# ray-project/ray

Hardware: AMD Instinct MI355X
Metric: train_samples_per_sec (higher is better)
Workload: dtype bf16; 1 GPU; model=llama3-8b, global_batch=8, micro_batch=8, seq_len=4096, parallelism=dp1, n_params=8030261248, bucket_mb=128, grad_checkpoint=False, harness=ray_amd.train.TorchTrainer

## Files before the change

ray_amd/csrc/hip/gemm_wgrad.hip:

```cpp
#include "common.h"
#include "fa_bwd_lds_layout.h"

typedef __attribute__((ext_vector_type(8))) __bf16 wg_bf16x8;
typedef __attribute__((ext_vector_type(16))) float wg_f32x16;
typedef __attribute__((ext_vector_type(2))) unsigned int wg_u32x2;
typedef __attribute__((ext_vector_type(4))) unsigned int wg_u32x4;

#define WG_STAGE 65536
#define WG_HALF 16384
#define WG_B 32768

template <int OFF>
DEV_INLINE wg_u32x2 wg_tr(unsigned addr) {
  wg_u32x2 v;
  asm volatile("ds_read_b64_tr_b16 %0, %1 offset:%2"
               : "=v"(v)
               : "v"(addr), "n"(OFF)
               : "memory");
  return v;
}

DEV_INLINE wg_bf16x8 wg_frag(wg_u32x2 lo, wg_u32x2 hi) {
  wg_u32x4 t = __builtin_shufflevector(lo, hi, 0, 1, 2, 3);
  return __builtin_bit_cast(wg_bf16x8, t);
}

DEV_INLINE void wg_stage_half(const char* g, unsigned lane_off, char* lds) {
  typedef const __attribute__((address_space(1))) void* gptr;
  typedef __attribute__((address_space(3))) void* lptr;
  __builtin_amdgcn_global_load_lds((gptr)(g + lane_off), (lptr)lds, 16, 0, 0);
  __builtin_amdgcn_global_load_lds((gptr)(g + 128 + lane_off),
                                   (lptr)(lds + 1024), 16, 0, 0);
}

struct WgRegs {
  wg_f32x16 acc[2][2][2];
  wg_u32x2 a[2][4][2];
  wg_u32x2 b[4][2];
};

template <int BASE, int S>
DEV_INLINE void wg_read_a1(WgRegs& r, unsigned a0, unsigned a1) {
  r.a[0][S][0] = wg_tr<BASE + 4096 * S>(a0);
  r.a[0][S][1] = wg_tr<BASE + 4096 * S + 2048>(a1);
  r.a[1][S][0] = wg_tr<BASE + 4096 * S + 512>(a0);
  r.a[1][S][1] = wg_tr<BASE + 4096 * S + 2048 + 512>(a1);
}
template <int BASE>
DEV_INLINE void wg_read_a(WgRegs& r, unsigned a0, unsigned a1) {
  wg_read_a1<BASE, 0>(r, a0, a1);
  wg_read_a1<BASE, 1>(r, a0, a1);
  wg_read_a1<BASE, 2>(r, a0, a1);
  wg_read_a1<BASE, 3>(r, a0, a1);
}

template <int BASE, int S>
DEV_INLINE void wg_read_b1(WgRegs& r, unsigned b0, unsigned b1) {
  r.b[S][0] = wg_tr<BASE + 4096 * S>(b0);
  r.b[S][1] = wg_tr<BASE + 4096 * S + 2048>(b1);
}
template <int BASE>
DEV_INLINE void wg_read_b(WgRegs& r, unsigned b0, unsigned b1) {
  wg_read_b1<BASE, 0>(r, b0, b1);
  wg_read_b1<BASE, 1>(r, b0, b1);
  wg_read_b1<BASE, 2>(r, b0, b1);
  wg_read_b1<BASE, 3>(r, b0, b1);
}

template <int HA, int HB>
DEV_INLINE void wg_mma(WgRegs& r) {
  asm volatile("s_waitcnt lgkmcnt(0)" ::: "memory");
  __builtin_amdgcn_sched_barrier(0);
  __builtin_amdgcn_s_barrier();
  __builtin_amdgcn_sched_barrier(0);
  __builtin_amdgcn_s_setprio(1);
#pragma unroll
  for (int s = 0; s < 4; ++s) {
    const wg_bf16x8 bf = wg_frag(r.b[s][0], r.b[s][1]);
#pragma unroll
    for (int i = 0; i < 2; ++i)
      r.acc[HA][HB][i] = __builtin_amdgcn_mfma_f32_32x32x16_bf16(
          wg_frag(r.a[i][s][0], r.a[i][s][1]), bf, r.acc[HA][HB][i], 0, 0, 0);
  }
  __builtin_amdgcn_s_setprio(0);
  __builtin_amdgcn_sched_barrier(0);
  __builtin_amdgcn_s_barrier();
  __builtin_amdgcn_sched_barrier(0);
}

template <int ST, bool NEXT_B0, bool NEXT2, int VMC>
DEV_INLINE void wg_tile(WgRegs& r, const unsigned (&ra)[2][2],
                        const unsigned (&rb)[2][2], char* lds_w, const char* gA,
                        const char* gB, unsigned la, unsigned lb,
                        long long tileA, long long tileB, int t) {
  constexpr int S = ST * WG_STAGE;
  constexpr int O = (ST ^ 1) * WG_STAGE;
  wg_read_a<0>(r, ra[ST][0], ra[ST][1]);
  wg_read_b<0>(r, rb[ST][0], rb[ST][1]);
  if (NEXT_B0)
    wg_stage_half(gB + (t + 1) * tileB, lb, lds_w + O + WG_B);
  wg_mma<0, 0>(r);
  wg_read_b<WG_HALF>(r, rb[ST][0], rb[ST][1]);
  if (NEXT2) wg_stage_half(gA + (t + 2) * tileA, la, lds_w + S);
  wg_mma<0, 1>(r);
  wg_read_a<WG_HALF>(r, ra[ST][0], ra[ST][1]);
  if (NEXT2)
    wg_stage_half(gB + (t + 2) * tileB + 256, lb, lds_w + S + WG_B + WG_HALF);
  wg_mma<1, 1>(r);
  wg_read_b<0>(r, rb[ST][0], rb[ST][1]);
  if (NEXT2)
    wg_stage_half(gA + (t + 2) * tileA + 256, la, lds_w + S + WG_HALF);
  if (VMC == 6) asm volatile("s_waitcnt vmcnt(6)" ::: "memory");
  if (VMC == 0) asm volatile("s_waitcnt vmcnt(0)" ::: "memory");
  wg_mma<1, 0>(r);
}

template <bool STAGGER>
__global__ __launch_bounds__(512) void gemm_wgrad_bf16(
    const short* __restrict__ dy0, const short* __restrict__ dy1,
    const short* __restrict__ x, short* __restrict__ out0,
    short* __restrict__ out1, int M, long long ldy, long long ldx,
    long long ldo, int NT, int nt0, int KT) {
  __shared__ __attribute__((aligned(1024))) char smem[2 * WG_STAGE];

  const int tid = threadIdx.x;
  const int w = __builtin_amdgcn_readfirstlane(tid >> 6);
  const int lane = tid & 63;
  const int wr = w >> 2, wc = w & 3;

  int tn, tk;
  {
    const int nwg = NT * KT;
    const int orig = blockIdx.x;
    const int xcd = orig & 7;
    const int q = nwg >> 3, rr = nwg & 7;
    const int id = (xcd < rr ? xcd * (q + 1) : rr * (q + 1) + (xcd - rr) * q) +
                   (orig >> 3);
    const int per = 8 * KT;
    const int grp = id / per;
    const int first = grp * 8;
    const int gsz = min(NT - first, 8);
    const int in = id - grp * per;
    tn = first + in % gsz;
    tk = in / gsz;
  }
  const bool p1 = tn >= nt0;
  const short* dy = p1 ? dy1 : dy0;
  short* out = p1 ? out1 : out0;
  const int tn_l = p1 ? tn - nt0 : tn;

  const char* gA = reinterpret_cast<const char*>(dy + (long long)tn_l * 256);
  const char* gB = reinterpret_cast<const char*>(x + (long long)tk * 256);
  const long long tileA = 64 * ldy * 2, tileB = 64 * ldx * 2;

  unsigned la, lb;
  {
    const int r7 = (lane >> 2) & 7;
    const int xo = 2 * (w & 1) + (r7 >> 2);
    const int ch = 4 * (lane >> 5) + ((lane & 3) ^ xo);
    const int row = 8 * w + r7;
    la = (unsigned)(row * (int)ldy * 2 + 16 * ch);
    lb = (unsigned)(row * (int)ldx * 2 + 16 * ch);
  }
  char* const lds_w = smem + 2048 * w;

  const unsigned sm0 = (unsigned)(size_t)(
      (__attribute__((address_space(3))) char*)smem);
  unsigned ra[2][2], rb[2][2];
#pragma unroll
  for (int mm = 0; mm < 2; ++mm) {
    const unsigned tb = sm0 + 2 * fb6_tbase(lane, mm);
    ra[0][mm] = tb + 1024 * wr;
    ra[1][mm] = tb + 1024 * wr + WG_STAGE;
    rb[0][mm] = tb + 512 * wc + WG_B;
    rb[1][mm] = tb + 512 * wc + WG_B + WG_STAGE;
  }

  WgRegs r;
#pragma unroll
  for (int a = 0; a < 2; ++a)
#pragma unroll
    for (int b = 0; b < 2; ++b)
#pragma unroll
      for (int i = 0; i < 2; ++i) r.acc[a][b][i] = wg_f32x16{};

  const int nt = M >> 6;

  wg_stage_half(gA, la, lds_w);
  wg_stage_half(gB, lb, lds_w + WG_B);
  wg_stage_half(gB + 256, lb, lds_w + WG_B + WG_HALF);
  wg_stage_half(gA + 256, la, lds_w + WG_HALF);
  wg_stage_half(gA + tileA, la, lds_w + WG_STAGE);
  wg_stage_half(gB + tileB + 256, lb, lds_w + WG_STAGE + WG_B + WG_HALF);
  wg_stage_half(gA + tileA + 256, la, lds_w + WG_STAGE + WG_HALF);
  asm volatile("s_waitcnt vmcnt(6)" ::: "memory");
  __builtin_amdgcn_s_barrier();
  __builtin_amdgcn_sched_barrier(0);
  if (STAGGER && wr) __builtin_amdgcn_s_barrier();
  __builtin_amdgcn_sched_barrier(0);

  int t = 0;
  for (; t < nt - 2; t += 2) {
    wg_tile<0, true, true, 6>(r, ra, rb, lds_w, gA, gB, la, lb, tileA, tileB,
                              t);
    wg_tile<1, true, true, 6>(r, ra, rb, lds_w, gA, gB, la, lb, tileA, tileB,
                              t + 1);
  }
  wg_tile<0, true, false, 0>(r, ra, rb, lds_w, gA, gB, la, lb, tileA, tileB,
                             t);
  wg_tile<1, false, false, -1>(r, ra, rb, lds_w, gA, gB, la, lb, tileA, tileB,
                               t + 1);
  if (STAGGER && !wr) __builtin_amdgcn_s_barrier();
  __builtin_amdgcn_sched_barrier(0);

  short* const ep = reinterpret_cast<short*>(smem);
  const int hi = lane >> 5, c32 = lane & 31;
#pragma unroll
  for (int ha = 0; ha < 2; ++ha) {
#pragma unroll
    for (int hb = 0; hb < 2; ++hb)
#pragma unroll
      for (int i = 0; i < 2; ++i)
#pragma unroll
        for (int g = 0; g < 16; ++g) {
          const int row = 64 * wr + 32 * i + (g & 3) + 8 * (g >> 2) + 4 * hi;
          const int col = 128 * hb + 32 * wc + c32;
          ep[row * 256 + col] =
              __builtin_bit_cast(short, (__bf16)r.acc[ha][hb][i][g]);
        }
    __syncthreads();
#pragma unroll
    for (int it = 0; it < 8; ++it) {
      const int c = tid + 512 * it;
      const int row = c >> 5, ch = c & 31;
      const short8 v = *reinterpret_cast<const short8*>(ep + row * 256 + 8 * ch);
      *reinterpret_cast<short8*>(
          out + ((long long)tn_l * 256 + 128 * ha + row) * ldo +
          (long long)tk * 256 + 8 * ch) = v;
    }
    __syncthreads();
  }
}
```

ray_amd/csrc/ops.hip:

```cpp
#include <torch/extension.h>
#include <ATen/hip/HIPContext.h>

#include "hip/rmsnorm.hip"
#include "hip/elementwise.hip"
#include "hip/rl_scans.hip"
#include "hip/cross_entropy.hip"
#include "hip/flash_attn_v5.hip"
#include "hip/flash_attn_v7.hip"
#include "hip/fa_bwd_prep.hip"
#include "hip/fa_bwd_v3.hip"
#include "hip/fa_bwd_dq_v5.hip"
#include "hip/fa_bwd_dkv_v6.hip"
#include "hip/gemv.hip"
#include "hip/paged_attn.hip"
#include "hip/paged_attn_prefill.hip"
#include "hip/gemm_wgrad.hip"

#define CHECK_IN(x)                                                     \
  TORCH_CHECK(x.is_cuda(), #x " must be on GPU");                       \
  TORCH_CHECK(x.is_contiguous(), #x " must be contiguous")

static inline hipStream_t cur_stream() {
  return at::hip::getCurrentHIPStream().stream();
}
// ... 273 lines not shown
              "paged cache must be [num_pages, Hkv, 16, D] matching q/k");
  return fp8;
}

static bool check_paged_attn(const at::Tensor& k_cache,
                             const at::Tensor& v_cache,
                             const at::Tensor& block_table, int B, int Hq,
                             int D, double k_scale, double v_scale, int* Hkv) {
  TORCH_CHECK(D == 64 || D == 128, "paged_attn: head_dim must be 64 or 128");
  TORCH_CHECK(k_cache.dim() == 4, "k_cache must be [num_pages, Hkv, 16, D]");
  *Hkv = (int)k_cache.size(1);
  const bool fp8 = check_paged_cache(k_cache, v_cache, *Hkv, D, k_scale,
                                     v_scale);
  TORCH_CHECK(*Hkv >= 1 && Hq % *Hkv == 0, "GQA requires Hq % Hkv == 0");
  const int rep = Hq / *Hkv;
  TORCH_CHECK(rep == 1 || rep == 2 || rep == 4 || rep == 8,
              "paged_attn: Hq/Hkv must be 1, 2, 4 or 8");
  TORCH_CHECK(block_table.dim() == 2 && block_table.size(0) == B &&
              block_table.size(1) >= 1,
              "block_table must be [B, max_pages]");
  return fp8;
}

static void launch_paged_reduce(const at::Tensor& ws, at::Tensor& out, int B,
                                int Hq, int D, int S) {
  const float* ws_o = ws.data_ptr<float>();
  const float* ws_ml = ws_o + (long long)B * Hq * S * D;
  hipLaunchKernelGGL(paged_attn_reduce_bf16, dim3(Hq, B), dim3(D), 0,
                     cur_stream(), ws_o, ws_ml, (short*)out.data_ptr(), Hq, S,
                     D);
}

at::Tensor paged_attn_reduce(at::Tensor workspace, int64_t B, int64_t Hq,
                             int64_t D, int64_t num_splits) {
  CHECK_IN(workspace);
  TORCH_CHECK(workspace.scalar_type() == at::kFloat, "workspace must be fp32");
  TORCH_CHECK(D == 64 || D == 128, "paged_attn: head_dim must be 64 or 128");
  TORCH_CHECK(B >= 1 && B <= 65535 && Hq >= 1 && Hq <= 65535 &&
              num_splits >= 1, "paged_attn_reduce: bad B/Hq/num_splits");
  TORCH_CHECK(workspace.numel() >= B * Hq * num_splits * (D + 2),
              "paged_attn: workspace too small");
  auto out = at::empty({B, Hq, D}, workspace.options().dtype(at::kBFloat16));
  launch_paged_reduce(workspace, out, (int)B, (int)Hq, (int)D,
                      (int)num_splits);
  return out;
}

template <int D, int REP, bool FP8, int EPL>
static void launch_paged_decode(const at::Tensor& q, const at::Tensor& kc,
                                const at::Tensor& vc, const at::Tensor& bt,
                                const at::Tensor& sl, at::Tensor& out,
                                float* ws_o, float* ws_ml, int S, int Hkv,
                                float k_scale, float v_scale) {
  int B = (int)q.size(0);
  hipLaunchKernelGGL((paged_attn_decode_kernel<D, REP, FP8, EPL>),
                     dim3(S, Hkv, B), dim3(256), 0, cur_stream(),
                     (const short*)q.data_ptr(), (const void*)kc.data_ptr(),
                     (const void*)vc.data_ptr(), bt.data_ptr<int>(),
                     sl.data_ptr<int>(), (short*)out.data_ptr(), ws_o, ws_ml,
                     Hkv, (int)kc.size(0), (int)bt.size(1),
                     1.4426950408889634f / sqrtf((float)D) * k_scale,
                     v_scale);
}

at::Tensor paged_attn_decode(at::Tensor q, at::Tensor k_cache,
                             at::Tensor v_cache, at::Tensor block_table,
                             at::Tensor seq_lens, int64_t num_splits,
                             c10::optional<at::Tensor> workspace,
                             double k_scale, double v_scale) {
  CHECK_IN(q);
  CHECK_I32(block_table);
  CHECK_I32(seq_lens);
  TORCH_CHECK(q.scalar_type() == at::kBFloat16, "q must be bf16");
  TORCH_CHECK(q.dim() == 3, "q must be [B, Hq, D]");
  int B = (int)q.size(0), Hq = (int)q.size(1), D = (int)q.size(2);
  int Hkv;
  const bool fp8 = check_paged_attn(k_cache, v_cache, block_table, B, Hq, D,
                                    k_scale, v_scale, &Hkv);
  int rep = Hq / Hkv;
  TORCH_CHECK(seq_lens.dim() == 1 && seq_lens.size(0) == B,
              "seq_lens must be [B]");
  TORCH_CHECK(B >= 1 && B <= 65535 && Hkv <= 65535,
              "paged_attn: B and Hkv must fit a grid dimension");
  int S = (int)num_splits;
  TORCH_CHECK(num_splits >= 1 && num_splits <= 1024,
              "paged_attn: num_splits must be 1..1024");
  auto out = at::empty({B, Hq, D}, q.options());
  at::Tensor ws;
  float *ws_o = nullptr, *ws_ml = nullptr;
  if (S > 1) {
    long long need = (long long)B * Hq * S * (D + 2);
    if (workspace.has_value()) {
      ws = *workspace;
      CHECK_IN(ws);
      TORCH_CHECK(ws.scalar_type() == at::kFloat && ws.numel() >= need,
                  "paged_attn: workspace must be fp32 with >= B*Hq*S*(D+2) "
                  "elements");
    } else {
      ws = at::empty({need}, q.options().dtype(at::kFloat));
    }
    ws_o = ws.data_ptr<float>();
    ws_ml = ws_o + (long long)B * Hq * S * D;
  }
#define PA_LAUNCH(DD, RR)                                                   \
  if (fp8)                                                                  \
    launch_paged_decode<DD, RR, true, PA_FP8_EPL>(                          \
        q, k_cache, v_cache, block_table, seq_lens, out, ws_o, ws_ml, S,    \
        Hkv, (float)k_scale, (float)v_scale);                               \
  else                                                                      \
    launch_paged_decode<DD, RR, false, 8>(q, k_cache, v_cache, block_table, \
                                          seq_lens, out, ws_o, ws_ml, S,    \
                                          Hkv, 1.f, 1.f)
#define PA_REP(DD)                                                          \
  switch (rep) {                                                            \
    case 1: PA_LAUNCH(DD, 1); break;                                        \
    case 2: PA_LAUNCH(DD, 2); break;                                        \
    case 4: PA_LAUNCH(DD, 4); break;                                        \
    default: PA_LAUNCH(DD, 8); break;                                       \
  }
  if (D == 64) { PA_REP(64) } else { PA_REP(128) }
#undef PA_REP
#undef PA_LAUNCH
  if (S > 1) launch_paged_reduce(ws, out, B, Hq, D, S);
  return out;
}

at::Tensor paged_attn_prefill(at::Tensor q, at::Tensor k_cache,
                              at::Tensor v_cache, at::Tensor block_table,
                              at::Tensor ctx_lens, at::Tensor q_lens,
                              double k_scale, double v_scale) {
  CHECK_IN(q);
  CHECK_I32(block_table);
  CHECK_I32(ctx_lens);
  CHECK_I32(q_lens);
  TORCH_CHECK(q.scalar_type() == at::kBFloat16, "q must be bf16");
  TORCH_CHECK(q.dim() == 4, "q must be [B, Tq, Hq, D]");
  TORCH_CHECK(aligned16(q), "paged_attn_prefill: q must be 16-byte aligned");
  int B = (int)q.size(0), Hq = (int)q.size(2), D = (int)q.size(3);
  int Hkv;
  const bool fp8 = check_paged_attn(k_cache, v_cache, block_table, B, Hq, D,
                                    k_scale, v_scale, &Hkv);
  TORCH_CHECK(fp8 || (aligned16(k_cache) && aligned16(v_cache)),
              "paged_attn_prefill: caches must be 16-byte aligned");
  TORCH_CHECK(block_table.size(1) <= (1 << 26),
              "paged_attn_prefill: block table too wide");
  TORCH_CHECK(ctx_lens.dim() == 1 && ctx_lens.size(0) == B &&
              q_lens.dim() == 1 && q_lens.size(0) == B,
              "ctx_lens and q_lens must be [B]");
  TORCH_CHECK(q.size(1) >= 1 && q.size(1) <= (1 << 26),
              "paged_attn_prefill: Tq must be 1..2^26");
  int Tq = (int)q.size(1);
  TORCH_CHECK(B >= 1 && B <= 65535 && Hq <= 65535,
              "paged_attn_prefill: B and Hq must fit a grid dimension");
  auto out = at::empty_like(q);
  const long long blocks128 = (long long)((Tq + 127) / 128) * Hq * B;
  const int waves = blocks128 >= PP_WIDE_TILE_BLOCKS ? 8 : 4;
  dim3 grid((Tq + 32 * waves - 1) / (32 * waves), Hq, B);
#define PP_LAUNCH_T(DD, WW, FP8)                                             \
  hipLaunchKernelGGL((paged_attn_prefill_kernel<DD, WW, FP8>), grid,        \
                     dim3(64 * WW), 0, cur_stream(),                        \
                     (const short*)q.data_ptr(),                            \
                     (const void*)k_cache.data_ptr(),                       \
                     (const void*)v_cache.data_ptr(),                       \
                     block_table.data_ptr<int>(), ctx_lens.data_ptr<int>(), \
                     q_lens.data_ptr<int>(), (short*)out.data_ptr(), Tq,    \
                     Hq, Hkv, (int)k_cache.size(0),                         \
                     (int)block_table.size(1),                              \
                     1.0f / sqrtf((float)D) * (float)k_scale,               \
                     (float)v_scale)
#define PP_LAUNCH(DD, WW)                                                   \
  if (fp8) { PP_LAUNCH_T(DD, WW, true); } else { PP_LAUNCH_T(DD, WW, false); }
  if (D == 64) {
    if (waves == 4) { PP_LAUNCH(64, 4); } else { PP_LAUNCH(64, 8); }
  } else {
    if (waves == 4) { PP_LAUNCH(128, 4); } else { PP_LAUNCH(128, 8); }
  }
#undef PP_LAUNCH
#undef PP_LAUNCH_T
  return out;
}

static long long paged_row_stride(const at::Tensor& t, const char* name) {
  TORCH_CHECK(t.is_cuda(), name, " must be on GPU");
  TORCH_CHECK(t.scalar_type() == at::kBFloat16, name, " must be bf16");
  TORCH_CHECK(t.dim() == 3 && t.stride(2) == 1 && t.stride(1) == t.size(2),
              name, " must be [B, H, D] with a contiguous [H, D] tail");
  TORCH_CHECK(t.stride(0) % 8 == 0 && aligned16(t), name,
              " rows must be 16-byte aligned");
  return (long long)t.stride(0);
}

at::Tensor rope_append_paged(at::Tensor q, at::Tensor k, at::Tensor v,
                             at::Tensor cosT, at::Tensor sinT, at::Tensor pos,
                             at::Tensor block_table, at::Tensor k_cache,
                             at::Tensor v_cache, double k_scale,
                             double v_scale) {
  long long q_rs = paged_row_stride(q, "q");
  long long k_rs = paged_row_stride(k, "k");
  long long v_rs = paged_row_stride(v, "v");
  CHECK_IN(cosT); CHECK_IN(sinT);
  CHECK_I32(pos);
  CHECK_I32(block_table);
  int B = (int)q.size(0), Hq = (int)q.size(1), D = (int)q.size(2);
  int Hkv = (int)k.size(1);
  TORCH_CHECK(D == 64 || D == 128, "paged_attn: head_dim must be 64 or 128");
  TORCH_CHECK(k.size(0) == B && v.size(0) == B && k.size(2) == D &&
              v.size(2) == D && v.size(1) == Hkv,
              "q/k/v shapes disagree");
  const bool fp8 = check_paged_cache(k_cache, v_cache, Hkv, D, k_scale,
                                     v_scale);
  TORCH_CHECK(cosT.scalar_type() == at::kFloat &&
              sinT.scalar_type() == at::kFloat && cosT.dim() == 2 &&
              cosT.size(1) == D / 2 && sinT.sizes() == cosT.sizes(),
              "cosT/sinT must be fp32 [T, D/2]");
  TORCH_CHECK(pos.dim() == 1 && pos.size(0) == B, "pos must be [B]");
  TORCH_CHECK(block_table.dim() == 2 && block_table.size(0) == B &&
              block_table.size(1) >= 1,
              "block_table must be [B, max_pages]");
  auto q_rot = at::empty({B, Hq, D}, q.options());
  if (B == 0) return q_rot;
#define RA_LAUNCH(FP8)                                                      \
  hipLaunchKernelGGL(rope_append_paged_kernel<FP8>, dim3(B), dim3(256), 0,  \
                     cur_stream(), (const short*)q.data_ptr(),              \
                     (const short*)k.data_ptr(), (const short*)v.data_ptr(),\
                     q_rs, k_rs, v_rs, cosT.data_ptr<float>(),              \
                     sinT.data_ptr<float>(), pos.data_ptr<int>(),           \
                     block_table.data_ptr<int>(), k_cache.data_ptr(),       \
                     v_cache.data_ptr(), (short*)q_rot.data_ptr(), Hq, Hkv, \
                     D, (int)cosT.size(0), (int)k_cache.size(0),            \
                     (int)block_table.size(1), (float)(1.0 / k_scale),      \
                     (float)(1.0 / v_scale))
  if (fp8) { RA_LAUNCH(true); } else { RA_LAUNCH(false); }
#undef RA_LAUNCH
  return q_rot;
}

void kv_append_paged(at::Tensor k, at::Tensor v, int64_t pos0,
                     at::Tensor block_table_row, at::Tensor k_cache,
                     at::Tensor v_cache, double k_scale, double v_scale) {
  long long k_rs = paged_row_stride(k, "k");
  long long v_rs = paged_row_stride(v, "v");
  CHECK_I32(block_table_row);
  int Hkv = (int)k.size(1), D = (int)k.size(2);
  TORCH_CHECK(D == 64 || D == 128, "paged_attn: head_dim must be 64 or 128");
  TORCH_CHECK(v.sizes() == k.sizes(), "k/v shapes disagree");
  const bool fp8 = check_paged_cache(k_cache, v_cache, Hkv, D, k_scale,
                                     v_scale);
  TORCH_CHECK(block_table_row.dim() == 1 && block_table_row.size(0) >= 1,
              "block_table_row must be [max_pages]");
  TORCH_CHECK(pos0 >= 0 && pos0 < (1ll << 31) && k.size(0) < (1ll << 31),
              "kv_append_paged: pos0 and T must be in 0..2^31");
  int T = (int)k.size(0);
  if (T == 0) return;
#define KA_LAUNCH(FP8)                                                      \
  hipLaunchKernelGGL(kv_append_paged_kernel<FP8>, dim3(T), dim3(128), 0,    \
                     cur_stream(), (const short*)k.data_ptr(),              \
                     (const short*)v.data_ptr(), k_rs, v_rs,                \
                     block_table_row.data_ptr<int>(), (int)pos0,            \
                     k_cache.data_ptr(), v_cache.data_ptr(), Hkv, D,        \
                     (int)k_cache.size(0), (int)block_table_row.size(0),    \
                     (float)(1.0 / k_scale), (float)(1.0 / v_scale))
  if (fp8) { KA_LAUNCH(true); } else { KA_LAUNCH(false); }
#undef KA_LAUNCH
}


static long long wgrad_operand(const at::Tensor& t, const char* name) {
  TORCH_CHECK(t.is_cuda(), name, " must be on GPU");
  TORCH_CHECK(t.scalar_type() == at::kBFloat16, name, " must be bf16");
  TORCH_CHECK(t.dim() == 2 && t.stride(1) == 1 && t.stride(0) >= t.size(1),
              name, " must be 2-D with unit column stride");
  TORCH_CHECK(t.stride(0) % 8 == 0 && aligned16(t), name,
              " rows must be 16-byte aligned");
  TORCH_CHECK(t.size(1) % 256 == 0 && t.size(1) >= 256, name,
              ": columns must be a multiple of 256");
  return (long long)t.stride(0);
}

static void launch_wgrad(const at::Tensor& dy0, const at::Tensor& dy1,
                         const at::Tensor& x, at::Tensor& out0,
                         at::Tensor& out1, int problems) {
  const long long ldy = wgrad_operand(dy0, "dy");
  const long long ldx = wgrad_operand(x, "x");
  const long long ldo = wgrad_operand(out0, "out");
  const long long M = dy0.size(0), N = dy0.size(1), K = x.size(1);
  TORCH_CHECK(x.size(0) == M && M >= 128 && M % 128 == 0,
              "gemm_wgrad: dy and x need the same number of rows, a "
              "multiple of 128");
  TORCH_CHECK(out0.size(0) == N && out0.size(1) == K,
              "gemm_wgrad: out must be [N, K]");
  TORCH_CHECK(ldy * 64 < (1ll << 30) && ldx * 64 < (1ll << 30),
              "gemm_wgrad: row stride too large");
  if (problems == 2) {
    TORCH_CHECK(wgrad_operand(dy1, "dy1") == ldy && dy1.size(0) == M &&
                    dy1.size(1) == N,
                "gemm_wgrad: grouped dy operands must match");
    TORCH_CHECK(wgrad_operand(out1, "out1") == ldo && out1.size(0) == N &&
                    out1.size(1) == K,
                "gemm_wgrad: grouped outputs must match");
  }
  const int nt0 = (int)(N / 256), KT = (int)(K / 256);
  const int NT = nt0 * problems;
  TORCH_CHECK((long long)NT * KT < (1ll << 31), "gemm_wgrad: grid too large");
#define WGRAD_LAUNCH(ST)                                                     \
  hipLaunchKernelGGL(gemm_wgrad_bf16<ST>, dim3((unsigned)(NT * KT)),         \
                     dim3(512), 0, cur_stream(),                             \
                     (const short*)dy0.data_ptr(),                           \
                     (const short*)dy1.data_ptr(),                           \
                     (const short*)x.data_ptr(), (short*)out0.data_ptr(),    \
                     (short*)out1.data_ptr(), (int)M, ldy, ldx, ldo, NT,     \
                     nt0, KT)
  if (getenv("RAY_AMD_WGRAD_NO_STAGGER") != nullptr) {
    WGRAD_LAUNCH(false);
  } else {
    WGRAD_LAUNCH(true);
  }
#undef WGRAD_LAUNCH
}

at::Tensor gemm_wgrad(at::Tensor dy, at::Tensor x,
                      c10::optional<at::Tensor> out) {
  at::Tensor o = out.has_value()
                     ? *out
                     : at::empty({dy.size(1), x.size(1)}, dy.options());
  launch_wgrad(dy, dy, x, o, o, 1);
  return o;
}

std::vector<at::Tensor> gemm_wgrad_grouped(at::Tensor dy0, at::Tensor dy1,
                                           at::Tensor x) {
  auto o0 = at::empty({dy0.size(1), x.size(1)}, dy0.options());
  auto o1 = at::empty_like(o0);
  launch_wgrad(dy0, dy1, x, o0, o1, 2);
  return {o0, o1};
}


void adamw_step(at::Tensor p, at::Tensor g, at::Tensor m, at::Tensor v,
                at::Tensor master, double lr, double beta1, double beta2,
                double eps, double wd, int64_t step, double grad_scale) {
  CHECK_IN(p); CHECK_IN(g); CHECK_IN(m); CHECK_IN(v);
  long long n = p.numel();
  float bc1 = 1.f - powf((float)beta1, (float)step);
  float bc2 = 1.f - powf((float)beta2, (float)step);
  if (p.scalar_type() == at::kBFloat16) {
    CHECK_IN(master);
    hipLaunchKernelGGL(adamw_step_bf16, dim3(grid_for(n)), dim3(256), 0,
                       cur_stream(), (short*)p.data_ptr(),
                       (const short*)g.data_ptr(), m.data_ptr<float>(),
                       v.data_ptr<float>(), master.data_ptr<float>(), n,
                       (float)lr, (float)beta1, (float)beta2, (float)eps,
                       (float)wd, bc1, bc2, (float)grad_scale);
  } else {
    hipLaunchKernelGGL(adamw_step_f32, dim3(grid_for(n)), dim3(256), 0,
                       cur_stream(), p.data_ptr<float>(),
                       g.data_ptr<float>(), m.data_ptr<float>(),
                       v.data_ptr<float>(), n, (float)lr, (float)beta1,
                       (float)beta2, (float)eps, (float)wd, bc1, bc2,
                       (float)grad_scale);
  }
}


std::vector<at::Tensor> gae(at::Tensor rewards, at::Tensor values,
                            at::Tensor cont, double gamma, double lam) {
  CHECK_IN(rewards); CHECK_IN(values); CHECK_IN(cont);
  int T = (int)rewards.size(0);
  int B = (int)rewards.size(1);
  TORCH_CHECK(values.size(0) == T + 1, "values must be [T+1, B]");
  auto adv = at::empty_like(rewards);
  auto vt = at::empty_like(rewards);
  hipLaunchKernelGGL(gae_scan_f32, dim3((B + 255) / 256), dim3(256), 0,
                     cur_stream(), rewards.data_ptr<float>(),
                     values.data_ptr<float>(), cont.data_ptr<float>(),
                     adv.data_ptr<float>(), vt.data_ptr<float>(), T, B,
                     (float)gamma, (float)lam);
  return {adv, vt};
}

std::vector<at::Tensor> vtrace(at::Tensor log_rhos, at::Tensor rewards,
                               at::Tensor values, at::Tensor cont,
                               double gamma, double rho_clip, double c_clip,
                               double rho_pg_clip) {
  CHECK_IN(log_rhos); CHECK_IN(rewards); CHECK_IN(values); CHECK_IN(cont);
  int T = (int)rewards.size(0);
  int B = (int)rewards.size(1);
  auto vs = at::empty_like(rewards);
  auto pg = at::empty_like(rewards);
  hipLaunchKernelGGL(vtrace_scan_f32, dim3((B + 255) / 256), dim3(256), 0,
                     cur_stream(), log_rhos.data_ptr<float>(),
                     rewards.data_ptr<float>(), values.data_ptr<float>(),
                     cont.data_ptr<float>(), vs.data_ptr<float>(),
                     pg.data_ptr<float>(), T, B, (float)gamma,
                     (float)rho_clip, (float)c_clip, (float)rho_pg_clip);
  return {vs, pg};
}


at::Tensor img_normalize(at::Tensor in, at::Tensor mean, at::Tensor inv_std) {
  CHECK_IN(in); CHECK_IN(mean); CHECK_IN(inv_std);
  TORCH_CHECK(in.scalar_type() == at::kByte && in.dim() == 4);
  long long N = in.size(0);
  int H = (int)in.size(1), W = (int)in.size(2), C = (int)in.size(3);
  auto out = at::empty({N, C, H, W}, in.options().dtype(at::kBFloat16));
  long long total = in.numel();
  hipLaunchKernelGGL(img_norm_u8_bf16, dim3(grid_for(total)), dim3(256), 0,
                     cur_stream(), in.data_ptr<unsigned char>(),
                     (short*)out.data_ptr(), mean.data_ptr<float>(),
                     inv_std.data_ptr<float>(), N, H, W, C);
  return out;
}


static void ce_check(const at::Tensor& logits, const at::Tensor& target) {
  CHECK_IN(logits); CHECK_IN(target);
  TORCH_CHECK(logits.scalar_type() == at::kBFloat16, "ce: logits must be bf16");
  TORCH_CHECK(target.scalar_type() == at::kInt, "ce: target must be int32");
  TORCH_CHECK(logits.dim() == 2 && logits.size(1) >= 1 &&
              logits.size(1) < (1ll << 31), "ce: logits must be [N, V]");
  TORCH_CHECK(target.dim() == 1 && target.size(0) == logits.size(0),
              "ce: target must be [N]");
  TORCH_CHECK(logits.size(1) % 8 != 0 || aligned16(logits),
              "ce: logits must be 16-byte aligned");
}

std::vector<at::Tensor> ce_fwd(at::Tensor logits, at::Tensor target) {
  ce_check(logits, target);
  long long N = logits.size(0);
  int V = (int)logits.size(1);
  auto loss = at::empty({N}, logits.options().dtype(at::kFloat));
  auto mx = at::empty({N}, logits.options().dtype(at::kFloat));
  auto lse = at::empty({N}, logits.options().dtype(at::kFloat));
  hipLaunchKernelGGL(ce_fwd_bf16, dim3((unsigned)N), dim3(256), 0,
                     cur_stream(), (const short*)logits.data_ptr(),
                     target.data_ptr<int>(), loss.data_ptr<float>(),
                     mx.data_ptr<float>(), lse.data_ptr<float>(), N, V);
  return {loss, mx, lse};
}

at::Tensor ce_bwd(at::Tensor logits, at::Tensor target, at::Tensor mx,
                  at::Tensor lse, at::Tensor dloss) {
  ce_check(logits, target);
  CHECK_IN(mx); CHECK_IN(lse); CHECK_IN(dloss);
  long long N = logits.size(0);
  TORCH_CHECK(lse.scalar_type() == at::kFloat && lse.numel() == N &&
              dloss.scalar_type() == at::kFloat && dloss.numel() == N,
              "ce: lse and dloss must be fp32 [N]");
  int V = (int)logits.size(1);
  auto dl = at::empty_like(logits);
  hipLaunchKernelGGL(ce_bwd_bf16, dim3((unsigned)N), dim3(256), 0,
                     cur_stream(), (const short*)logits.data_ptr(),
                     target.data_ptr<int>(), mx.data_ptr<float>(),
                     lse.data_ptr<float>(), dloss.data_ptr<float>(),
                     (short*)dl.data_ptr(), N, V);
  return dl;
}


static inline int attn_layout(const at::Tensor& t, long long* rs) {
  if (t.stride(3) != 1) return -1;
  long long H = t.size(1), T = t.size(2), D = t.size(3);
  *rs = D;
  if (t.stride(2) == D && t.stride(1) == T * D && t.stride(0) == H * T * D)
    return 0;
  const long long r = t.stride(2);
  if (t.stride(1) != D || t.stride(0) != T * r || r < H * D) return -1;
  *rs = r;
  if (r == H * D) return 1;
  if (r % 8 == 0 && aligned16(t) && T * r < (1ll << 31) &&
      64 * r < (1ll << 30))
    return 1;
  return -1;
}

std::vector<at::Tensor> flash_attn_fwd(at::Tensor q, at::Tensor k,
                                        at::Tensor v, bool causal,
                                        int64_t q_offset, bool want_lse) {
  TORCH_CHECK(q.is_cuda() && k.is_cuda() && v.is_cuda(),
              "flash_attn tensors must be on GPU");
  long long q_rs, k_rs, v_rs;
  int bthd = attn_layout(q, &q_rs);
  TORCH_CHECK(bthd >= 0 && attn_layout(k, &k_rs) == bthd &&
                  attn_layout(v, &v_rs) == bthd && k_rs == v_rs,
              "q/k/v must share a BHTD-contiguous or BTHD-view layout");
  TORCH_CHECK(q.scalar_type() == at::kBFloat16, "q must be bf16");
  TORCH_CHECK(q.size(3) == 128, "head_dim must be 128");
  TORCH_CHECK(q.size(2) % 128 == 0, "T must be a multiple of 128 (pad)");
  int B = (int)q.size(0), Hq = (int)q.size(1), T = (int)q.size(2);
  int Hkv = (int)k.size(1), Tk = (int)k.size(2);
  TORCH_CHECK(Hq % Hkv == 0, "GQA requires Hq % Hkv == 0");
  TORCH_CHECK(!bthd || T % 256 == 0,
              "BTHD-view layout needs T % 256 == 0: only the 256-row "
              "kernel reads it");
  auto o = bthd
               ? at::empty({B, T, Hq, (int)q.size(3)}, q.options())
                     .permute({0, 2, 1, 3})
               : at::empty_like(q);
  const long long o_rs = bthd ? (long long)Hq * q.size(3) : q.size(3);
  at::Tensor lse;
  float* lse_ptr = nullptr;
  if (want_lse) {
    lse = at::empty({B, Hq, T}, q.options().dtype(at::kFloat));
    lse_ptr = lse.data_ptr<float>();
  }
  float scale = 1.0f / sqrtf((float)q.size(3));
  const short* qp = (const short*)q.data_ptr();
  const short* kp = (const short*)k.data_ptr();
  const short* vp = (const short*)v.data_ptr();
  short* op = (short*)o.data_ptr();
  const int c = causal ? 1 : 0, qo = (int)q_offset;
  if (T % 256 == 0)
    hipLaunchKernelGGL(flash_attn_fwd_v7_bf16, dim3(T / 256, B * Hq),
                       dim3(512), 0, cur_stream(), qp, kp, vp, op, lse_ptr,
                       B, Hq, Hkv, T, Tk, c, qo, scale, bthd, (int)q_rs,
                       (int)o_rs, (int)k_rs);
  else
    hipLaunchKernelGGL(flash_attn_fwd_v5_bf16, dim3(T / 128, B * Hq),
                       dim3(256), 0, cur_stream(), qp, kp, vp, op, lse_ptr,
                       B, Hq, Hkv, T, Tk, c, qo, scale);
  if (want_lse) return {o, lse};
  return {o};
}

std::vector<at::Tensor> flash_attn_bwd(at::Tensor q, at::Tensor k,
                                        at::Tensor v, at::Tensor o,
                                        at::Tensor d_o, at::Tensor lse,
                                        bool causal,
                                        c10::optional<at::Tensor> dqkv) {
  TORCH_CHECK(q.is_cuda(), "flash_attn_bwd tensors must be on GPU");
  long long q_rs, k_rs, v_rs, o_rs, do_rs;
  int bthd = attn_layout(q, &q_rs);
  TORCH_CHECK(bthd >= 0 && attn_layout(k, &k_rs) == bthd &&
                  attn_layout(v, &v_rs) == bthd &&
                  attn_layout(o, &o_rs) == bthd &&
                  attn_layout(d_o, &do_rs) == bthd && k_rs == v_rs,
              "q/k/v/o/dO must share a BHTD or BTHD-view layout");
  TORCH_CHECK(q.scalar_type() == at::kBFloat16, "q must be bf16");
  TORCH_CHECK(q.size(3) == 128, "head_dim must be 128");
  TORCH_CHECK(q.size(2) % 128 == 0, "T must be a multiple of 128");
  TORCH_CHECK(q.size(2) == k.size(2),
              "bwd requires T == Tk (training self-attention)");
  int B = (int)q.size(0), Hq = (int)q.size(1), T = (int)q.size(2);
  int Hkv = (int)k.size(1);
  TORCH_CHECK(Hq % Hkv == 0, "GQA requires Hq % Hkv == 0");
  TORCH_CHECK(!bthd || T % 256 == 0,
              "BTHD-view layout needs T % 256 == 0: only the 256-row "
              "kernels read it");
  int D = (int)q.size(3);
  TORCH_CHECK(!bthd || (o_rs == (long long)Hq * D && do_rs == o_rs),
              "o and dO must be [B,T,Hq,D] storage in the BTHD-view layout");
  at::Tensor dq, dk, dv;
  long long dq_rs = q_rs, dkv_rs = k_rs;
  if (dqkv.has_value()) {
    const at::Tensor& g = *dqkv;
    const long long W = (long long)(Hq + 2 * Hkv) * D;
    TORCH_CHECK(bthd == 1, "dqkv needs q/k/v in the BTHD-view layout");
    TORCH_CHECK(g.is_cuda() && g.scalar_type() == at::kBFloat16 &&
                    g.dim() == 3 && g.size(0) == B && g.size(1) == T &&
                    g.size(2) == W,
                "dqkv must be bf16 [B, T, (Hq+2Hkv)*D] on the GPU");
    const long long r = g.stride(1);
    TORCH_CHECK(g.stride(2) == 1 && g.stride(0) == T * r && r >= W &&
                    r % 8 == 0 && aligned16(g) && T * r < (1ll << 31) &&
                    64 * r < (1ll << 30),
                "dqkv rows must be 16-byte aligned, at stride >= "
                "(Hq+2Hkv)*D with T * stride < 2^31");
    auto section = [&](long long col, int H) {
      return g.narrow(2, col, (long long)H * D)
          .view({B, T, H, D})
          .permute({0, 2, 1, 3});
    };
    dq = section(0, Hq);
    dk = section((long long)Hq * D, Hkv);
    dv = section((long long)(Hq + Hkv) * D, Hkv);
    dq_rs = dkv_rs = r;
  } else {
    auto mk_like = [&](const at::Tensor& t, int H) {
      return bthd
                 ? at::empty({B, T, H, D}, t.options()).permute({0, 2, 1, 3})
                 : at::empty_like(t);
    };
    dq = mk_like(q, Hq);
    dk = mk_like(k, Hkv);
    dv = mk_like(v, Hkv);
    if (bthd) {
      dq_rs = (long long)Hq * D;
      dkv_rs = (long long)Hkv * D;
    }
  }
  auto dsum = at::empty({B, Hq, T}, q.options().dtype(at::kFloat));
  float scale = 1.0f / sqrtf((float)q.size(3));
  long long rows = (long long)B * Hq * T;
  const short* qp = (const short*)q.data_ptr();
  const short* kp = (const short*)k.data_ptr();
  const short* vp = (const short*)v.data_ptr();
  const short* dop = (const short*)d_o.data_ptr();
  const float* lsep = lse.data_ptr<float>();
  float* dsp = dsum.data_ptr<float>();
  short* dqp = (short*)dq.data_ptr();
  short* dkp = (short*)dk.data_ptr();
  short* dvp = (short*)dv.data_ptr();
  const int c = causal ? 1 : 0;
  hipStream_t st = cur_stream();
  hipLaunchKernelGGL(fa_bwd_prep_bf16, dim3((rows + 3) / 4), dim3(256), 0,
                     st, dop, (const short*)o.data_ptr(), dsp, rows, Hq, T,
                     bthd);
  if (T % 256 == 0) {
    hipLaunchKernelGGL(fa_bwd_dq_v5_bf16, dim3(T / 256, B * Hq), dim3(512),
                       0, st, qp, kp, vp, dop, lsep, dsp, dqp, B, Hq, Hkv, T,
                       c, scale, bthd, (int)q_rs, (int)o_rs, (int)k_rs,
                       (int)dq_rs);
    hipLaunchKernelGGL(fa_bwd_dkv_v6_bf16, dim3(B * Hkv, T / 256), dim3(512),
                       0, st, qp, kp, vp, dop, lsep, dsp, dkp, dvp, B, Hq,
                       Hkv, T, c, scale, bthd, (int)q_rs, (int)o_rs, (int)k_rs,
                       (int)dkv_rs);
  } else {
    const dim3 blk(256);
    hipLaunchKernelGGL(fa_bwd_dq_v3_bf16, dim3(T / 128, B * Hq), blk, 0, st,
                       qp, kp, vp, dop, lsep, dsp, dqp, B, Hq, Hkv, T, c,
                       scale, 0);
    hipLaunchKernelGGL(fa_bwd_dkv_v3_bf16<false>, dim3(T / 128, B * Hkv), blk,
                       0, st, qp, kp, vp, dop, lsep, dsp, dvp, B, Hq, Hkv, T,
                       c, scale);
    hipLaunchKernelGGL(fa_bwd_dkv_v3_bf16<true>, dim3(T / 128, B * Hkv), blk,
                       0, st, qp, kp, vp, dop, lsep, dsp, dkp, B, Hq, Hkv, T,
                       c, scale);
  }
  return {dq, dk, dv};
}

void rope_qk_inplace(at::Tensor qkv, at::Tensor cosT, at::Tensor sinT,
                     int64_t n_heads, int64_t n_kv_heads, int64_t sign) {
  CHECK_IN(cosT); CHECK_IN(sinT);
  TORCH_CHECK(qkv.is_cuda() && qkv.scalar_type() == at::kBFloat16 &&
                  qkv.dim() == 3,
              "rope_qk_inplace: qkv must be a bf16 [B, T, W] GPU tensor");
  TORCH_CHECK(sign == 1 || sign == -1, "rope_qk_inplace: sign must be +-1");
  TORCH_CHECK(n_heads >= 1 && n_kv_heads >= 1 &&
                  qkv.size(2) % (n_heads + 2 * n_kv_heads) == 0,
              "rope_qk_inplace: W must be (Hq + 2 Hkv) * D");
  const long long B = qkv.size(0), T = qkv.size(1), W = qkv.size(2);
  const int D = (int)(W / (n_heads + 2 * n_kv_heads));
  const long long rs = qkv.stride(1);
  TORCH_CHECK(D > 0 && D % 16 == 0, "rope_qk_inplace: D must be a multiple "
                                    "of 16");
  TORCH_CHECK(qkv.stride(2) == 1 && rs >= W && rs % 8 == 0 &&
                  (B == 1 || qkv.stride(0) == T * rs) && aligned16(qkv),
              "rope_qk_inplace: rows must be 16-byte aligned with a uniform "
              "stride >= W");
  TORCH_CHECK(cosT.scalar_type() == at::kFloat &&
                  sinT.scalar_type() == at::kFloat && cosT.dim() == 2 &&
                  cosT.size(0) >= T && cosT.size(1) == D / 2 &&
                  sinT.sizes() == cosT.sizes() && aligned16(cosT) &&
                  aligned16(sinT),
              "rope_qk_inplace: cosT/sinT must be 16-byte-aligned fp32 "
              "[>= T, D/2]");
  const int n_rot = (int)(n_heads + n_kv_heads);
  const long long total = B * T * n_rot * (D / 16);
  if (total == 0) return;
  hipLaunchKernelGGL(rope_qk_inplace_bf16, dim3(grid_for(total)), dim3(256), 0,
                     cur_stream(), (short*)qkv.data_ptr(),
                     cosT.data_ptr<float>(), sinT.data_ptr<float>(), B * T, D,
                     n_rot, (int)T, (int)sign, rs);
}

PYBIND11_MODULE(TORCH_EXTENSION_NAME, m) {
  m.def("flash_attn_fwd", &flash_attn_fwd);
  m.def("flash_attn_bwd", &flash_attn_bwd, py::arg("q"), py::arg("k"),
        py::arg("v"), py::arg("o"), py::arg("d_o"), py::arg("lse"),
        py::arg("causal"), py::arg("dqkv") = py::none());
  m.def("rope_qk_inplace", &rope_qk_inplace);
  m.def("rmsnorm_fwd", &rmsnorm_fwd);
  m.def("gemv", &gemv);
  m.def("gemm_wgrad", &gemm_wgrad, py::arg("dy"), py::arg("x"),
        py::arg("out") = py::none());
  m.def("gemm_wgrad_grouped", &gemm_wgrad_grouped);
  m.def("paged_attn_decode", &paged_attn_decode, py::arg("q"),
        py::arg("k_cache"), py::arg("v_cache"), py::arg("block_table"),
        py::arg("seq_lens"), py::arg("num_splits"),
        py::arg("workspace") = py::none(), py::arg("k_scale") = 1.0,
        py::arg("v_scale") = 1.0);
  m.def("paged_attn_reduce", &paged_attn_reduce);
  m.def("rope_append_paged", &rope_append_paged, py::arg("q"), py::arg("k"),
        py::arg("v"), py::arg("cosT"), py::arg("sinT"), py::arg("pos"),
        py::arg("block_table"), py::arg("k_cache"), py::arg("v_cache"),
        py::arg("k_scale") = 1.0, py::arg("v_scale") = 1.0);
  m.def("kv_append_paged", &kv_append_paged);
  m.def("paged_attn_prefill", &paged_attn_prefill, py::arg("q"),
        py::arg("k_cache"), py::arg("v_cache"), py::arg("block_table"),
        py::arg("ctx_lens"), py::arg("q_lens"), py::arg("k_scale") = 1.0,
        py::arg("v_scale") = 1.0);
  m.def("rmsnorm_bwd", &rmsnorm_bwd);
  m.def("rmsnorm_bwd_two_pass", &rmsnorm_bwd_two_pass);
  m.def("rmsnorm_bwd_res", &rmsnorm_bwd_res, py::arg("dy"), py::arg("x"),
        py::arg("w"), py::arg("inv"), py::arg("g_res") = py::none(),
        py::arg("grid") = 0);
  m.def("add_rmsnorm_fwd", &add_rmsnorm_fwd);
  m.def("swiglu_fwd", &swiglu_fwd);
  m.def("swiglu_bwd", &swiglu_bwd);
  m.def("rope_apply", &rope_apply);
  m.def("adamw_step", &adamw_step);
  m.def("gae", &gae);
  m.def("vtrace", &vtrace);
  m.def("img_normalize", &img_normalize);
  m.def("ce_fwd", &ce_fwd);
  m.def("ce_bwd", &ce_bwd);
  m.attr("gfx_arch") = "gfx950";
  m.attr("rmsnorm_bwd_grid") = RMS_BWD_GRID;
}
```

Baseline: 5.602 samples/s.

## Add XCD-aware 8x4 tile rasterization and keep B0 fragment registers across MMA phases

Adds a new block-to-tile mapping that hands each XCD contiguous 32-block chunks laid out as 8x4 rectangles of output tiles, with remainder handling, so co-resident blocks share L2 data. Adds a second B-fragment register set so the first B half is kept in registers instead of being re-read from LDS before the last MMA phase. Both are on by default (arms=3) and can be toggled by environment variables, and a host helper exposing the tile map is added for testing. The extra B registers raise VGPR pressure.

Measured after the change: 5.652 samples/s, median of 6. No clear change (+0.9%).

```diff
diff --git a/ray_amd/csrc/hip/gemm_wgrad.hip b/ray_amd/csrc/hip/gemm_wgrad.hip
--- a/ray_amd/csrc/hip/gemm_wgrad.hip
+++ b/ray_amd/csrc/hip/gemm_wgrad.hip
@@ -1,5 +1,6 @@
 #include "common.h"
 #include "fa_bwd_lds_layout.h"
+#include "gemm_wgrad_map.h"
 
 typedef __attribute__((ext_vector_type(8))) __bf16 wg_bf16x8;
 typedef __attribute__((ext_vector_type(16))) float wg_f32x16;
@@ -36,7 +37,7 @@
 struct WgRegs {
   wg_f32x16 acc[2][2][2];
   wg_u32x2 a[2][4][2];
-  wg_u32x2 b[4][2];
+  wg_u32x2 b[2][4][2];
 };
 
 template <int BASE, int S>
@@ -54,20 +55,20 @@
   wg_read_a1<BASE, 3>(r, a0, a1);
 }
 
-template <int BASE, int S>
+template <int BASE, int BS, int S>
 DEV_INLINE void wg_read_b1(WgRegs& r, unsigned b0, unsigned b1) {
-  r.b[S][0] = wg_tr<BASE + 4096 * S>(b0);
-  r.b[S][1] = wg_tr<BASE + 4096 * S + 2048>(b1);
-}
-template <int BASE>
+  r.b[BS][S][0] = wg_tr<BASE + 4096 * S>(b0);
+  r.b[BS][S][1] = wg_tr<BASE + 4096 * S + 2048>(b1);
+}
+template <int BASE, int BS>
 DEV_INLINE void wg_read_b(WgRegs& r, unsigned b0, unsigned b1) {
-  wg_read_b1<BASE, 0>(r, b0, b1);
-  wg_read_b1<BASE, 1>(r, b0, b1);
-  wg_read_b1<BASE, 2>(r, b0, b1);
-  wg_read_b1<BASE, 3>(r, b0, b1);
-}
-
-template <int HA, int HB>
+  wg_read_b1<BASE, BS, 0>(r, b0, b1);
+  wg_read_b1<BASE, BS, 1>(r, b0, b1);
+  wg_read_b1<BASE, BS, 2>(r, b0, b1);
+  wg_read_b1<BASE, BS, 3>(r, b0, b1);
+}
+
+template <int HA, int HB, int BS>
 DEV_INLINE void wg_mma(WgRegs& r) {
   asm volatile("s_waitcnt lgkmcnt(0)" ::: "memory");
   __builtin_amdgcn_sched_barrier(0);
@@ -76,7 +77,7 @@
   __builtin_amdgcn_s_setprio(1);
 #pragma unroll
   for (int s = 0; s < 4; ++s) {
-    const wg_bf16x8 bf = wg_frag(r.b[s][0], r.b[s][1]);
+    const wg_bf16x8 bf = wg_frag(r.b[BS][s][0], r.b[BS][s][1]);
 #pragma unroll
     for (int i = 0; i < 2; ++i)
       r.acc[HA][HB][i] = __builtin_amdgcn_mfma_f32_32x32x16_bf16(
@@ -88,34 +89,35 @@
   __builtin_amdgcn_sched_barrier(0);
 }
 
-template <int ST, bool NEXT_B0, bool NEXT2, int VMC>
+template <int ST, bool NEXT_B0, bool NEXT2, int VMC, bool KEEP_B0>
 DEV_INLINE void wg_tile(WgRegs& r, const unsigned (&ra)[2][2],
                         const unsigned (&rb)[2][2], char* lds_w, const char* gA,
                         const char* gB, unsigned la, unsigned lb,
                         long long tileA, long long tileB, int t) {
   constexpr int S = ST * WG_STAGE;
   constexpr int O = (ST ^ 1) * WG_STAGE;
+  constexpr int B0S = KEEP_B0 ? 1 : 0;
   wg_read_a<0>(r, ra[ST][0], ra[ST][1]);
-  wg_read_b<0>(r, rb[ST][0], rb[ST][1]);
+  wg_read_b<0, B0S>(r, rb[ST][0], rb[ST][1]);
   if (NEXT_B0)
     wg_stage_half(gB + (t + 1) * tileB, lb, lds_w + O + WG_B);
-  wg_mma<0, 0>(r);
-  wg_read_b<WG_HALF>(r, rb[ST][0], rb[ST][1]);
+  wg_mma<0, 0, B0S>(r);
+  wg_read_b<WG_HALF, 0>(r, rb[ST][0], rb[ST][1]);
   if (NEXT2) wg_stage_half(gA + (t + 2) * tileA, la, lds_w + S);
-  wg_mma<0, 1>(r);
+  wg_mma<0, 1, 0>(r);
   wg_read_a<WG_HALF>(r, ra[ST][0], ra[ST][1]);
   if (NEXT2)
     wg_stage_half(gB + (t + 2) * tileB + 256, lb, lds_w + S + WG_B + WG_HALF);
-  wg_mma<1, 1>(r);
-  wg_read_b<0>(r, rb[ST][0], rb[ST][1]);
+  wg_mma<1, 1, 0>(r);
+  if (!KEEP_B0) wg_read_b<0, 0>(r, rb[ST][0], rb[ST][1]);
   if (NEXT2)
     wg_stage_half(gA + (t + 2) * tileA + 256, la, lds_w + S + WG_HALF);
   if (VMC == 6) asm volatile("s_waitcnt vmcnt(6)" ::: "memory");
   if (VMC == 0) asm volatile("s_waitcnt vmcnt(0)" ::: "memory");
-  wg_mma<1, 0>(r);
-}
-
-template <bool STAGGER>
+  wg_mma<1, 0, B0S>(r);
+}
+
+template <bool STAGGER, int ARMS>
 __global__ __launch_bounds__(512) void gemm_wgrad_bf16(
     const short* __restrict__ dy0, const short* __restrict__ dy1,
     const short* __restrict__ x, short* __restrict__ out0,
@@ -129,7 +131,9 @@
   const int wr = w >> 2, wc = w & 3;
 
   int tn, tk;
-  {
+  if (ARMS & 1) {
+    wgrad_tile_of(blockIdx.x, NT, KT, tn, tk);
+  } else {
     const int nwg = NT * KT;
     const int orig = blockIdx.x;
     const int xcd = orig & 7;
@@ -185,6 +189,7 @@
       for (int i = 0; i < 2; ++i) r.acc[a][b][i] = wg_f32x16{};
 
   const int nt = M >> 6;
+  constexpr bool KB0 = (ARMS & 2) != 0;
 
   wg_stage_half(gA, la, lds_w);
   wg_stage_half(gB, lb, lds_w + WG_B);
@@ -201,15 +206,15 @@
 
   int t = 0;
   for (; t < nt - 2; t += 2) {
-    wg_tile<0, true, true, 6>(r, ra, rb, lds_w, gA, gB, la, lb, tileA, tileB,
-                              t);
-    wg_tile<1, true, true, 6>(r, ra, rb, lds_w, gA, gB, la, lb, tileA, tileB,
-                              t + 1);
-  }
-  wg_tile<0, true, false, 0>(r, ra, rb, lds_w, gA, gB, la, lb, tileA, tileB,
-                             t);
-  wg_tile<1, false, false, -1>(r, ra, rb, lds_w, gA, gB, la, lb, tileA, tileB,
-                               t + 1);
+    wg_tile<0, true, true, 6, KB0>(r, ra, rb, lds_w, gA, gB, la, lb, tileA,
+                                   tileB, t);
+    wg_tile<1, true, true, 6, KB0>(r, ra, rb, lds_w, gA, gB, la, lb, tileA,
+                                   tileB, t + 1);
+  }
+  wg_tile<0, true, false, 0, KB0>(r, ra, rb, lds_w, gA, gB, la, lb, tileA,
+                                  tileB, t);
+  wg_tile<1, false, false, -1, KB0>(r, ra, rb, lds_w, gA, gB, la, lb, tileA,
+                                    tileB, t + 1);
   if (STAGGER && !wr) __builtin_amdgcn_s_barrier();
   __builtin_amdgcn_sched_barrier(0);
 
diff --git a/ray_amd/csrc/hip/gemm_wgrad_map.h b/ray_amd/csrc/hip/gemm_wgrad_map.h
--- /dev/null
+++ b/ray_amd/csrc/hip/gemm_wgrad_map.h
@@ -0,0 +1,40 @@
+#pragma once
+#include <hip/hip_runtime.h>
+
+__host__ __device__ inline void wgrad_tile_of(int b, int NT, int KT, int& tn,
+                                              int& tk) {
+  const int nwg = NT * KT;
+  const int x = b & 7, j = b >> 3;
+  const int R = nwg >> 8, T = nwg & 255;
+  int p;
+  if (j < 32 * R) {
+    p = 256 * (j >> 5) + 32 * x + (j & 31);
+  } else {
+    const int q = T >> 3, rr = T & 7;
+    const int start = x < rr ? x * (q + 1) : rr * (q + 1) + (x - rr) * q;
+    p = 256 * R + start + (j - 32 * R);
+  }
+  const int NF = NT >> 3, nr = NT & 7;
+  const int KF = KT >> 2, kr = KT & 3;
+  const int full = 32 * NF * KF;
+  if (p < full) {
+    const int rect = p >> 5, idx = p & 31;
+    tn = 8 * (rect / KF) + (idx & 7);
+    tk = 4 * (rect % KF) + (idx >> 3);
+    return;
+  }
+  p -= full;
+  const int right = 8 * NF * kr;
+  if (p < right) {
+    const int per = 8 * kr;
+    const int idx = p % per;
+    tn = 8 * (p / per) + (idx & 7);
+    tk = 4 * KF + (idx >> 3);
+    return;
+  }
+  p -= right;
+  const int per = 4 * nr;
+  const int idx = p % per;
+  tn = 8 * NF + idx % nr;
+  tk = 4 * (p / per) + idx / nr;
+}
diff --git a/ray_amd/csrc/ops.hip b/ray_amd/csrc/ops.hip
--- a/ray_amd/csrc/ops.hip
+++ b/ray_amd/csrc/ops.hip
@@ -599,20 +599,41 @@
   const int nt0 = (int)(N / 256), KT = (int)(K / 256);
   const int NT = nt0 * problems;
   TORCH_CHECK((long long)NT * KT < (1ll << 31), "gemm_wgrad: grid too large");
-#define WGRAD_LAUNCH(ST)                                                     \
-  hipLaunchKernelGGL(gemm_wgrad_bf16<ST>, dim3((unsigned)(NT * KT)),         \
+#define WGRAD_LAUNCH(ST, ARMS)                                               \
+  hipLaunchKernelGGL((gemm_wgrad_bf16<ST, ARMS>), dim3((unsigned)(NT * KT)), \
                      dim3(512), 0, cur_stream(),                             \
                      (const short*)dy0.data_ptr(),                           \
                      (const short*)dy1.data_ptr(),                           \
                      (const short*)x.data_ptr(), (short*)out0.data_ptr(),    \
                      (short*)out1.data_ptr(), (int)M, ldy, ldx, ldo, NT,     \
                      nt0, KT)
-  if (getenv("RAY_AMD_WGRAD_NO_STAGGER") != nullptr) {
-    WGRAD_LAUNCH(false);
-  } else {
-    WGRAD_LAUNCH(true);
-  }
+#define WGRAD_ARMS(ARMS)                                 \
+  if (getenv("RAY_AMD_WGRAD_NO_STAGGER") != nullptr) {   \
+    WGRAD_LAUNCH(false, ARMS);                           \
+  } else {                                               \
+    WGRAD_LAUNCH(true, ARMS);                            \
+  }
+  int arms = 3;
+  if (getenv("RAY_AMD_WGRAD_V1") != nullptr) arms = 0;
+  if (const char* a = getenv("RAY_AMD_WGRAD_ARMS")) arms = (a[0] - '0') & 3;
+  switch (arms) {
+    case 0: WGRAD_ARMS(0); break;
+    case 1: WGRAD_ARMS(1); break;
+    case 2: WGRAD_ARMS(2); break;
+    default: WGRAD_ARMS(3); break;
+  }
+#undef WGRAD_ARMS
 #undef WGRAD_LAUNCH
+}
+
+at::Tensor wgrad_tile_map(int64_t NT, int64_t KT) {
+  TORCH_CHECK(NT >= 1 && KT >= 1 && NT * KT < (1ll << 31),
+              "wgrad_tile_map: bad grid");
+  at::Tensor t = at::empty({NT * KT, 2}, at::kInt);
+  int* p = t.data_ptr<int>();
+  for (int b = 0; b < (int)(NT * KT); ++b)
+    wgrad_tile_of(b, (int)NT, (int)KT, p[2 * b], p[2 * b + 1]);
+  return t;
 }
 
 at::Tensor gemm_wgrad(at::Tensor dy, at::Tensor x,
@@ -972,6 +993,7 @@
   m.def("gemm_wgrad", &gemm_wgrad, py::arg("dy"), py::arg("x"),
         py::arg("out") = py::none());
   m.def("gemm_wgrad_grouped", &gemm_wgrad_grouped);
+  m.def("wgrad_tile_map", &wgrad_tile_map, py::arg("NT"), py::arg("KT"));
   m.def("paged_attn_decode", &paged_attn_decode, py::arg("q"),
         py::arg("k_cache"), py::arg("v_cache"), py::arg("block_table"),
         py::arg("seq_lens"), py::arg("num_splits"),
```
